# line/Human-Interaction-Generation

Measured on AMD Instinct MI355X. Metric: denoiser-fwd frames/s @ B=64·T=196, higher is better.
Workload: dtype f32; 1 GPU; MotionTransformer forward incl. the per-call cross-attention text side, BASELINE config 2: B=64/GPU T=196 F=150 d=512 L=8 H=8 ff=1024 N=77 Lt=256, linear attention, text embeddings supplied (CLIP stubbed); parallelism=dp1

## Files before the change

human-interaction-generation_amd/csrc/gemm_wsp32.hip:

```cpp
#include <stdlib.h>

#include <type_traits>

#include "hig_common.h"
#include "hig_host.h"

namespace {

typedef float f32x4 __attribute__((ext_vector_type(4)));
typedef int p32_i32x4 __attribute__((ext_vector_type(4)));

constexpr int P32_MAXSEG = HIG_P32_MAXSEG;
struct Wsp32Args {
  const float* X; int64_t ldx;
  const float* W; int64_t ldy;
  float* C; int64_t ldc;
  const float* res; int64_t ldr;
  float* aux; int64_t ldaux;
  const float* bias;
  int I, J;
  int ntiles;
  int nseg, seg_p0[P32_MAXSEG], seg_np[P32_MAXSEG];
  float* stats_out;
  const float* stats_in;
// ... 27 lines not shown
#if defined(__HIP_DEVICE_COMPILE__)
  const p32_i32x4 d = __builtin_bit_cast(p32_i32x4, v);
  if constexpr (POL == 1) __builtin_amdgcn_raw_buffer_store_b128(d, rs, byte_off, 0, 16);
  else __builtin_amdgcn_raw_buffer_store_b128(d, rs, byte_off, 0, 0);
#endif
}
__device__ __forceinline__ f32x4 p32_lds16(unsigned addr) {
  f32x4 v;
  asm volatile("ds_read_b128 %0, %1" : "=v"(v) : "v"(addr));
  return v;
}
typedef float f32x2_t __attribute__((ext_vector_type(2)));
__device__ __forceinline__ f32x2_t p32_lds8(unsigned addr) {
  f32x2_t v;
  asm volatile("ds_read_b64 %0, %1" : "=v"(v) : "v"(addr));
  return v;
}
__device__ __forceinline__ float p32_erf_abs(float ax, float& ex) {
  const float t = __builtin_amdgcn_rcpf(fmaf(ax, 0.3275911f * 0.70710678118654752440f, 1.0f));
  float p = fmaf(t, 1.061405429f, -1.453152027f);
  p = fmaf(t, p, 1.421413741f);
  p = fmaf(t, p, -0.284496736f);
  p = fmaf(t, p, 0.254829592f);
  p *= t;
  const float zz = ax * (0.70710678118654752440f * 1.2011224087864498f);
  ex = __builtin_amdgcn_exp2f(-(zz * zz));
  return fmaf(-p, ex, 1.0f);
}
__device__ __forceinline__ float p32_gelu(float x) {
  float ex;
  const float e = p32_erf_abs(fabsf(x), ex);
  return 0.5f * x * (1.0f + copysignf(e, x));
}
__device__ __forceinline__ float p32_dgelu(float z) {
  float ex;
  const float e = p32_erf_abs(fabsf(z), ex);
  return fmaf(z * 0.39894228040143267794f, ex, 0.5f + copysignf(0.5f * e, z));
}
__host__ __device__ constexpr bool p32_has_bias(int e) { return e == HIG_EPI_BIAS || e == HIG_EPI_BIAS_GELU || e == HIG_EPI_BIAS_RES; }
__host__ __device__ constexpr bool p32_has_res(int e) { return e == HIG_EPI_BIAS_RES || e == HIG_EPI_RES || e == HIG_EPI_DGELU; }

template <int PPR, int COUNT, int STEP>
__device__ __forceinline__ void p32_dma_rows([[maybe_unused]] __amdgpu_buffer_rsrc_t rs, int ld, int row0, int rmax, [[maybe_unused]] char* dst, int first, int lane) {
#pragma unroll
  for (int q = 0; q < COUNT; ++q) {
    const int n = first + STEP * q;
    const int r = n / PPR, part = n % PPR;
    [[maybe_unused]] const int voff = 16 * (lane ^ (r & 15));
    [[maybe_unused]] const int soff = min(row0 + r, rmax) * ld * 4 + part * 1024;
#if defined(__HIP_DEVICE_COMPILE__)
    __builtin_amdgcn_raw_ptr_buffer_load_lds(rs, (__attribute__((address_space(3))) void*)(dst + n * 1024), 16, voff, soff, 0, 0);
#endif
  }
}

template <int KW, int EPI, int XT, bool AUX, int POL, bool DIAG>
__global__ __launch_bounds__(512, 2) void gemm_wsp32_kernel(const Wsp32Args a) {
  constexpr int BM = 16;
  constexpr int ROWB = KW * 4;
  constexpr int XBUF = BM * ROWB;
  constexpr int RING = 128 * 1024;
  constexpr int NXB = RING / XBUF;
#ifndef P32_LOOK
#define P32_LOOK 1
#endif
  constexpr int LOOK = NXB - 1 < P32_LOOK ? NXB - 1 : P32_LOOK;
  constexpr bool NEED_CNT = NXB < LOOK + 2;
  constexpr int NH = KW / 256;
  constexpr int NC = 4 / NH;
  constexpr int BN = 32 * NC;
  constexpr int NKS = 16;
  constexpr int XS = 3;
  constexpr int RS = XS + 1;
  constexpr int HROW = BN * 4 + 16;
  constexpr int HPL = BM * HROW;
  constexpr int HBUF = NH * HPL;
  constexpr int RBUF = 4096, NRB = 3;
  constexpr int LBUF = 1024;
  constexpr int OFF_H = RING;
  constexpr int OFF_R = OFF_H + 2 * HBUF;
  constexpr int OFF_L = OFF_R + NRB * RBUF;
  constexpr int SMEM = OFF_L + (XT == 2 ? NRB * LBUF : 0);
  constexpr int OFF_C = OFF_H + BN * 4;
  constexpr int NSL = BN / 16;
  constexpr int PPR = ROWB / 1024;
  constexpr int NXI = BM * PPR / 4;
  constexpr int QPR = BN / 4;
  constexpr int RPP = QPR > 16 ? 64 / QPR : 4;
  constexpr int NPASS = 4 / RPP;
  constexpr bool HAS_RES = p32_has_res(EPI);
  static_assert(SMEM <= 160 * 1024, "LDS budget");
  static_assert(XT == 0 || (KW == 512 && ((XT == 1 && EPI == HIG_EPI_BIAS_RES) || (XT == 2 && EPI == HIG_EPI_BIAS))), "LayerNorm fold: K = 512, producer = BIAS_RES, consumer = BIAS");
  static_assert(!AUX || EPI == HIG_EPI_BIAS_GELU, "aux output: GELU epilogue only");
  static_assert(KW != 256 || (!HAS_RES && XT == 0 && !AUX), "K = 256 (the text-side key/value projection): plain / bias epilogue only");
  static_assert(NKS % RS == 0, "the ring index of a k-step is its number modulo RS in every tile");
  __shared__ __attribute__((aligned(1024))) char smem[160 * 1024];
  char* const sX = smem;
  char* const sH = smem + OFF_H;
  [[maybe_unused]] char* const sR = smem + OFF_R;
  [[maybe_unused]] char* const sL = smem + OFF_L;
  int* const scnt = reinterpret_cast<int*>(smem + OFF_C);

  const int tid = threadIdx.x, lane = tid & 63;
  const int wave = __builtin_amdgcn_readfirstlane(tid >> 6);
  const int w = (blockIdx.x & 7) * 32 + (blockIdx.x >> 3);
  constexpr bool W_BEHIND = KW == 512;
  static_assert(W_BEHIND ? (NSL == NXB && OFF_H + XBUF <= 160 * 1024) : NSL <= NXB, "weight slices fit");
  auto wslice = [&](int s) -> char* { return (W_BEHIND && s == NSL - 1) ? sH : sX + s * XBUF; };
  auto stamp = [&]([[maybe_unused]] int k) {
    if constexpr (!DIAG) return;
    if (a.stamps && (tid == 0 || tid == 256)) {
      unsigned long long tm;
      asm volatile("s_memtime %0\n\ts_waitcnt lgkmcnt(0)" : "=s"(tm)::"memory");
      a.stamps[(size_t)(tid ? 4096 : 0) + (size_t)blockIdx.x * 16 + k] = tm;
    }
  };
  stamp(0);

  if (wave < 4) {
    const int c = wave / NH, h = wave % NH;
    const int ln = lane & 15, kq = lane >> 4;
    int xo[4];
#pragma unroll
    for (int q = 0; q < 4; ++q) xo[q] = ln * ROWB + 1024 * h + 16 * ((4 * q + kq) ^ ln);
    const unsigned scnt_lds = (unsigned)(size_t)(__attribute__((address_space(3))) int*)scnt;
    const unsigned sx_lds = (unsigned)(size_t)(__attribute__((address_space(3))) char*)sX;
    char* const hmine = sH + h * HPL + ln * HROW + (32 * c + 4 * kq) * 4;

    for (int seg = 0; seg < a.nseg; ++seg) {
      const int nps = a.seg_np[seg], G = 256 / nps;
      const int rg = w / nps;
      const int tb = (int)((int64_t)rg * a.ntiles / G), te = (int)((int64_t)(rg + 1) * a.ntiles / G);
      const int nt = te - tb;
      p32_barrier();
      p32_barrier();
      f32x4 wf[NKS][2];
#pragma unroll
      for (int cb = 0; cb < 2; ++cb) {
        const char* wb = wslice(2 * c + cb);
#pragma unroll
        for (int ks = 0; ks < NKS; ++ks) wf[ks][cb] = *reinterpret_cast<const f32x4*>(wb + xo[ks & 3] + 256 * (ks >> 2));
      }
      p32_barrier();
      if (NEED_CNT && tid == 0) *scnt = 0;
      if (seg == 0) stamp(1);

      f32x4 acc0[2], acc1[2];
      f32x4 ring[RS];
#pragma unroll
      for (int e = 0; e < 2; ++e) { acc0[e] = f32x4{0.f, 0.f, 0.f, 0.f}; acc1[e] = f32x4{0.f, 0.f, 0.f, 0.f}; }
      auto signal_reads_issued = [&]() {
        if (lane == 0) asm volatile("ds_add_u32 %0, %1" ::"v"(scnt_lds), "v"(1) : "memory");
      };
      auto step = [&](auto has_tail, auto has_main, f32x4(&aP)[2], f32x4(&aQ)[2], int i) {
        constexpr bool TAIL = decltype(has_tail)::value, MAIN = decltype(has_main)::value;
        if (DIAG && seg == 0 && i == 5) stamp(11);
        if constexpr (TAIL && MAIN) asm volatile("s_waitcnt lgkmcnt(%0)" ::"n"(NEED_CNT ? XS + 1 : XS) : "memory");
        else asm volatile("s_waitcnt lgkmcnt(0)" ::: "memory");
        __builtin_amdgcn_s_barrier();
        asm volatile("" ::: "memory");
        if (DIAG && seg == 0 && i < 9) stamp(2 + i);
        unsigned xa[4];
        const unsigned xb = sx_lds + ((i + NXB - 1) % NXB) * XBUF;
#pragma unroll
        for (int q = 0; q < 4; ++q) {
          xa[q] = xb + xo[q];
          asm volatile("" : "+v"(xa[q]));
        }
        auto dump = [&]() {
          char* hp = hmine + ((i - 1) & 1) * HBUF;
#pragma unroll
          for (int cb = 0; cb < 2; ++cb) {
            *reinterpret_cast<f32x4*>(hp + cb * 64) = aQ[cb];
            aQ[cb] = f32x4{0.f, 0.f, 0.f, 0.f};
          }
        };
#pragma unroll
        for (int s = 0; s < NKS; ++s) {
#pragma unroll
          for (int j = 0; j < 4; ++j) {
#pragma unroll
            for (int cb = 0; cb < 2; ++cb) {
              if (s < XS) {
                if constexpr (TAIL) aQ[cb] = __builtin_amdgcn_mfma_f32_16x16x4f32(wf[NKS - XS + s][cb][j], ring[(NKS - XS + s) % RS][j], aQ[cb], 0, 0, 0);
              } else {
                if constexpr (MAIN) aP[cb] = __builtin_amdgcn_mfma_f32_16x16x4f32(wf[s - XS][cb][j], ring[(s - XS) % RS][j], aP[cb], 0, 0, 0);
              }
            }
            if constexpr (MAIN) {
              if (j == 0) ring[s % RS] = *reinterpret_cast<const __attribute__((address_space(3))) f32x4*>(xa[s & 3] + 256 * (s >> 2));
            }
          }
          if constexpr (TAIL) { if (s == (MAIN ? XS + 1 : XS - 1)) dump(); }
          {
            const int cur = (s < XS ? NKS - XS + s : s - XS) % RS;
            if ((s < XS && TAIL) || (s >= XS && MAIN)) asm volatile("" ::"v"(ring[cur]));
          }
          __builtin_amdgcn_sched_barrier(0);
        }
        if constexpr (MAIN && NEED_CNT) signal_reads_issued();
      };
      using T = std::true_type;
      using F = std::false_type;
      step(F{}, T{}, acc0, acc1, 0);
      int i = 1;
      for (; i + 1 < nt; i += 2) {
        step(T{}, T{}, acc1, acc0, i);
        step(T{}, T{}, acc0, acc1, i + 1);
      }
      if (i < nt) {
        step(T{}, T{}, acc1, acc0, i);
        ++i;
      }
      if (nt & 1) step(T{}, F{}, acc1, acc0, nt);
      else step(T{}, F{}, acc0, acc1, nt);
      p32_barrier();
    }
    stamp(12);
    return;
  }

  const int sw = wave - 4;
  const unsigned scnt_lds_s = (unsigned)(size_t)(__attribute__((address_space(3))) int*)scnt;
  if (a.prio == 1) __builtin_amdgcn_s_setprio(1);
  else if (a.prio == 2) __builtin_amdgcn_s_setprio(2);
  else if (a.prio == 3) __builtin_amdgcn_s_setprio(3);
  const int cq = lane & (QPR - 1), rsub = (lane / QPR) % RPP;
  const bool act = lane < 4 * QPR;
  __amdgpu_buffer_rsrc_t rsX = __builtin_amdgcn_make_buffer_rsrc(const_cast<float*>(a.X), 0, (int)(((int64_t)(a.I - 1) * a.ldx + KW) * 4), 0x00020000);
  __amdgpu_buffer_rsrc_t rsW = __builtin_amdgcn_make_buffer_rsrc(const_cast<float*>(a.W), 0, (int)(((int64_t)(a.J - 1) * a.ldy + KW) * 4), 0x00020000);
  __amdgpu_buffer_rsrc_t rsC = __builtin_amdgcn_make_buffer_rsrc(a.C, 0, (int)(((int64_t)(a.I - 1) * a.ldc + a.J) * 4), 0x00020000);
  [[maybe_unused]] __amdgpu_buffer_rsrc_t rsA = __builtin_amdgcn_make_buffer_rsrc(AUX ? a.aux : a.C, 0, (int)(((int64_t)(a.I - 1) * (AUX ? a.ldaux : a.ldc) + a.J) * 4), 0x00020000);
  [[maybe_unused]] __amdgpu_buffer_rsrc_t rsR = __builtin_amdgcn_make_buffer_rsrc(const_cast<float*>(HAS_RES ? a.res : a.X), 0, (int)(((int64_t)(a.I - 1) * (HAS_RES ? a.ldr : a.ldx) + (HAS_RES ? a.J : KW)) * 4), 0x00020000);
  for (int seg = 0; seg < a.nseg; ++seg) {
    const int nps = a.seg_np[seg], G = 256 / nps;
    const int panel = a.seg_p0[seg] + w % nps, rg = w / nps;
    const int tb = (int)((int64_t)rg * a.ntiles / G), te = (int)((int64_t)(rg + 1) * a.ntiles / G);
    const int nt = te - tb;
    const int j0 = panel * BN;
    f32x4 bq = {0.f, 0.f, 0.f, 0.f}, cs = {0.f, 0.f, 0.f, 0.f};
    auto dma_x = [&](int t) { p32_dma_rows<PPR, NXI, 4>(rsX, (int)a.ldx, (tb + t) * BM, a.I - 1, sX + ((t + NXB - 1) % NXB) * XBUF, sw, lane); };
    auto dma_res = [&](int t) {
      if constexpr (HAS_RES) {
        [[maybe_unused]] const int voff = (min((tb + t) * BM + 4 * sw + rsub, a.I - 1) * (int)a.ldr + j0 + 4 * cq) * 4;
#if defined(__HIP_DEVICE_COMPILE__)
        __builtin_amdgcn_raw_ptr_buffer_load_lds(rsR, (__attribute__((address_space(3))) void*)(sR + (t % NRB) * RBUF + sw * 1024), 16, voff, 0, 0, 0);
#endif
      }
    };
    auto dma_stats = [&](int t) {
      if constexpr (XT == 2) {
        if (sw == 0) {
          const int i = min((tb + t) * BM + (lane >> 2), a.I - 1);
          __builtin_amdgcn_global_load_lds((const __attribute__((address_space(1))) void*)(a.stats_in + (int64_t)i * 16 + 4 * (lane & 3)),
                                           (__attribute__((address_space(3))) void*)(sL + (t % NRB) * LBUF), 16, 0, 0);
        }
      }
    };

    p32_barrier();
#pragma unroll
    for (int s = 0; s < NSL; ++s) p32_dma_rows<PPR, NXI, 4>(rsW, (int)a.ldy, j0 + 16 * s, a.J - 1, wslice(s), sw, lane);
    if constexpr (p32_has_bias(EPI)) asm volatile("global_load_dwordx4 %0, %1, off" : "=v"(bq) : "v"(a.bias + j0 + 4 * cq) : "memory");
    if constexpr (XT == 2) asm volatile("global_load_dwordx4 %0, %1, off" : "=v"(cs) : "v"(a.colsum + j0 + 4 * cq) : "memory");
    int pre = 0;
    if constexpr (W_BEHIND) { dma_x(0); pre = 1; asm volatile("s_waitcnt vmcnt(%2)" : "+v"(bq), "+v"(cs) : "n"(NXI) : "memory"); }
    else asm volatile("s_waitcnt vmcnt(0)" : "+v"(bq), "+v"(cs) :: "memory");
    p32_barrier();
    p32_barrier();
    for (int t = pre; t < LOOK && t < nt; ++t) dma_x(t);
    {
      const int later = (max(min(LOOK, nt), 1) - 1) * NXI;
      p32_wait_vm(later);
    }

    constexpr int NST = NPASS * (1 + (XT == 1 ? 1 : 0) + (AUX ? 1 : 0));
    const unsigned sh_lds = (unsigned)(size_t)(__attribute__((address_space(3))) char*)sH;
    [[maybe_unused]] const unsigned sr_lds = (unsigned)(size_t)(__attribute__((address_space(3))) char*)sR;
    [[maybe_unused]] const unsigned sl_lds = (unsigned)(size_t)(__attribute__((address_space(3))) char*)sL;
    auto epilogue = [&](int e) {
#pragma unroll
     for (int pass = 0; pass < NPASS; ++pass) {
      const int row = 4 * sw + RPP * pass + rsub;
      const unsigned hp = sh_lds + (e & 1) * HBUF + row * HROW + 16 * cq;
      f32x4 hh[NH];
#pragma unroll
      for (int p = 0; p < NH; ++p) hh[p] = p32_lds16(hp + p * HPL);
      [[maybe_unused]] f32x4 rr = {0.f, 0.f, 0.f, 0.f};
      if constexpr (HAS_RES) rr = p32_lds16(sr_lds + (e % NRB) * RBUF + sw * 1024 + lane * 16);
      [[maybe_unused]] f32x2_t ps = {0.f, 0.f};
      if constexpr (XT == 2) ps = p32_lds8(sl_lds + (e % NRB) * LBUF + row * 64 + 8 * (cq & 7));
      if constexpr (NH == 1) asm volatile("s_waitcnt lgkmcnt(0)" : "+v"(hh[0]), "+v"(rr), "+v"(ps));
      else if constexpr (NH == 2) asm volatile("s_waitcnt lgkmcnt(0)" : "+v"(hh[0]), "+v"(hh[1]), "+v"(rr), "+v"(ps));
      else asm volatile("s_waitcnt lgkmcnt(0)" : "+v"(hh[0]), "+v"(hh[1]), "+v"(hh[2]), "+v"(hh[3]), "+v"(rr), "+v"(ps));
      float v[4];
#pragma unroll
      for (int k = 0; k < 4; ++k) {
        v[k] = hh[0][k];
#pragma unroll
        for (int p = 1; p < NH; ++p) v[k] += hh[p][k];
      }
      if constexpr (XT == 2) {
        const bool mine = cq < 8;
        const float tot = row16_sum(mine ? ps.x : 0.f), m2 = row16_sum(mine ? ps.y : 0.f);
        const float mean = tot * (1.0f / 512.0f);
        const float d0 = fmaf(ps.x, 1.0f / 64.0f, -mean);
        const float between = row16_sum(mine ? d0 * d0 : 0.f);
        const float rstd = rsqrtf(fmaf(64.0f, between, m2) * (1.0f / 512.0f) + 1e-5f), mr = -mean * rstd;
#pragma unroll
        for (int k = 0; k < 4; ++k) v[k] = fmaf(v[k], rstd, mr * cs[k]);
      }
#pragma unroll
      for (int k = 0; k < 4; ++k) v[k] += bq[k];
      const int ig = min((tb + e) * BM + row, a.I - 1);
      if constexpr (AUX) { if (act && !(DIAG && (a.dbg & 4))) p32_store16<POL>(rsA, (ig * (int)a.ldaux + j0 + 4 * cq) * 4, f32x4{v[0], v[1], v[2], v[3]}); }
#pragma unroll
      for (int k = 0; k < 4; ++k) {
        if constexpr (EPI == HIG_EPI_BIAS_RES || EPI == HIG_EPI_RES) v[k] += rr[k];
        if constexpr (EPI == HIG_EPI_BIAS_GELU) v[k] = p32_gelu(v[k]);
        if constexpr (EPI == HIG_EPI_DGELU) v[k] *= p32_dgelu(rr[k]);
      }
      if (DIAG && (a.dbg & 4)) { asm volatile("" ::"v"(v[0]), "v"(v[1]), "v"(v[2]), "v"(v[3])); continue; }
      if (act) p32_store16<POL>(rsC, (ig * (int)a.ldc + j0 + 4 * cq) * 4, f32x4{v[0], v[1], v[2], v[3]});
      if constexpr (XT == 1) {
        const float sm = row16_sum((v[0] + v[1]) + (v[2] + v[3]));
        const float pm = sm * (1.0f / 64.0f);
        const float a0 = v[0] - pm, a1 = v[1] - pm, a2 = v[2] - pm, a3 = v[3] - pm;
        const float qq = row16_sum((a0 * a0 + a1 * a1) + (a2 * a2 + a3 * a3));
        if (cq == 0) *reinterpret_cast<float2*>(a.stats_out + ((int64_t)ig * (a.J >> 6) + panel) * 2) = make_float2(sm, qq);
      }
     }
    };

    auto dbg = [&](int bit) { return DIAG && (a.dbg & bit) != 0; };
    auto n_x = [&](int i) { return (i >= 0 && i + LOOK < nt && !(dbg(1) && i > 2)) ? NXI : 0; };
    auto n_r = [&](int i) { return (HAS_RES && i >= 0 && i < nt) ? 1 : 0; };
    auto n_s = [&](int i) { return (XT == 2 && i >= 0 && i < nt && sw == 0) ? 1 : 0; };
    auto n_st = [&](int i) { return (i >= 2 && i < nt + 2 && !dbg(6)) ? NST : 0; };
    for (int i = 0; i < nt + 2; ++i) {
      p32_barrier();
      if (DIAG && i == 4 && seg == 0) stamp(0);
      if (i < nt) { dma_res(i); dma_stats(i); }
      if (DIAG && i == 4 && seg == 0) stamp(4);
      if (n_x(i)) {
        if constexpr (NEED_CNT) {
          int seen;
          do {
            asm volatile("ds_read_b32 %0, %1\n\ts_waitcnt lgkmcnt(0)" : "=v"(seen) : "v"(scnt_lds_s) : "memory");
          } while (__builtin_amdgcn_readfirstlane(seen) < 4 * i);
        }
        dma_x(i + LOOK);
      }
      if (DIAG && i == 4 && seg == 0) stamp(1);
      if (i >= 2 && !dbg(2)) epilogue(i - 2);
      if (DIAG && i == 4 && seg == 0) stamp(2);
      if constexpr (LOOK == 1) p32_wait_vm(n_st(i));
// ... 82 lines not shown
```

human-interaction-generation_amd/csrc/linattn.hip:

```cpp
#include <stdlib.h>

#include "hig_host.h"

namespace {

constexpr int CH = 64;

template <int HD> struct Patch {
  static constexpr int PC = HD >= 128 ? 8 : HD >= 64 ? 4 : HD >= 32 ? 2 : 1;
  static constexpr int PL = PC;
  static constexpr int TL = HD / PL;
};

template <int HD>
__global__ __launch_bounds__(256) void ctx_kernel(const float* __restrict__ K,
                                                  const float* __restrict__ V, int64_t ld, int rows,
                                                  int H, const int64_t* __restrict__ length,
                                                  float* __restrict__ A, float* __restrict__ kstat) {
  constexpr int LDP = HD + 4;
  constexpr int PC = Patch<HD>::PC, PL = Patch<HD>::PL, TL = Patch<HD>::TL;
  constexpr int RG = 256 / HD;
  __shared__ __attribute__((aligned(16))) float sP[CH * LDP];
  __shared__ __attribute__((aligned(16))) float sV[CH * LDP];
  __shared__ float sred[256];
// ... 1606 lines not shown
        const float dv = acc[hh][tb][e] - mean;
        qd += dv * dv;
      }
  }
  qd += __shfl_xor(qd, 32, 64);
  if (kk == 0) red[1][wave][lr] = qd;
  __syncthreads();
  const float rstd = rsqrtf(((red[1][0][lr] + red[1][1][lr]) + (red[1][2][lr] + red[1][3][lr])) / (float)d + 1e-5f);
  TO* sO = reinterpret_cast<TO*>(smem_dyn);
  const int ldso = d + 16 / (int)sizeof(TO);
  const float* ssrow = ss + (int64_t)b * ss_ld;
#pragma unroll
  for (int hh = 0; hh < MAXHPW; ++hh) {
    if (hh >= HPW) break;
    const int h = wave * HPW + hh;
#pragma unroll
    for (int tb = 0; tb < TB; ++tb)
#pragma unroll
      for (int qq = 0; qq < 4; ++qq) {
        const int col = h * HD + 32 * tb + 8 * qq + 4 * kk;
        const float4 g4 = *reinterpret_cast<const float4*>(gamma + col), b4 = *reinterpret_cast<const float4*>(beta + col);
        const float4 sc = *reinterpret_cast<const float4*>(ssrow + col), sh = *reinterpret_cast<const float4*>(ssrow + shift_off + col);
        float4 o;
        o.x = apply_sty_act<TO>(((acc[hh][tb][4 * qq] - mean) * rstd * g4.x + b4.x) * (1.0f + sc.x) + sh.x);
        o.y = apply_sty_act<TO>(((acc[hh][tb][4 * qq + 1] - mean) * rstd * g4.y + b4.y) * (1.0f + sc.y) + sh.y);
        o.z = apply_sty_act<TO>(((acc[hh][tb][4 * qq + 2] - mean) * rstd * g4.z + b4.z) * (1.0f + sc.z) + sh.z);
        o.w = apply_sty_act<TO>(((acc[hh][tb][4 * qq + 3] - mean) * rstd * g4.w + b4.w) * (1.0f + sc.w) + sh.w);
        st4(sO + lr * ldso + col, o);
      }
  }
  __syncthreads();
  constexpr int EO = 16 / (int)sizeof(TO);
  const int c16 = d / EO;
  for (int idx = tid; idx < 32 * c16; idx += 256) {
    const int rr = idx / c16, ch = idx % c16;
    if (r0 + rr < rows)
      *reinterpret_cast<uint4*>(Out + ((int64_t)b * rows + r0 + rr) * ldo + EO * ch) =
          *reinterpret_cast<const uint4*>(sO + rr * ldso + EO * ch);
  }
}

template <typename TQ, typename TO>
int launch_apply_sty(const TQ* q, int64_t ldq, const float* A, const float* gamma, const float* beta, const float* ss,
                     int64_t ss_ld, int32_t shift_off, TO* o, int64_t ldo, int32_t B, int32_t rows, int32_t H, int32_t hd,
                     hipStream_t st) {
  const int nblk = (rows + 31) / 32;
  const int d = H * hd;
  const size_t wbuf = (size_t)32 * (hd + 4) > 4096 ? (size_t)32 * (hd + 4) : 4096;
  const size_t lds_main = 4 * wbuf * sizeof(float);
  const size_t lds_out = (size_t)32 * (d + 16 / sizeof(TO)) * sizeof(TO);
  const size_t lds = lds_main > lds_out ? lds_main : lds_out;
  constexpr bool HAS64 = !std::is_same<TQ, float>::value;
  static const int big_lds_rc = [] {
    hipError_t e1 = hipSuccess;
    if constexpr (HAS64)
      e1 = hipFuncSetAttribute(reinterpret_cast<const void*>(&apply_sty_kernel<64, TQ, TO>),
                               hipFuncAttributeMaxDynamicSharedMemorySize, 156 * 1024);
    hipError_t e2 = hipFuncSetAttribute(reinterpret_cast<const void*>(&apply_sty_kernel<128, TQ, TO>),
                                        hipFuncAttributeMaxDynamicSharedMemorySize, 156 * 1024);
    return (e1 == hipSuccess && e2 == hipSuccess) ? 0 : 1;
  }();
  if (big_lds_rc != 0 || lds > 156 * 1024)
    return hig_set_error(HIG_EHIP, "hig_linattn_apply_sty: cannot reserve %zu bytes of LDS", lds);
  if (hd == 64) {
    if constexpr (HAS64)
      hipLaunchKernelGGL((apply_sty_kernel<64, TQ, TO>), dim3(B * nblk), dim3(256), lds, st, q, ldq, A, gamma, beta, ss, ss_ld,
                         shift_off, o, ldo, rows, H, nblk);
    else
      return hig_set_error(HIG_EUNSUPPORTED, "hig_linattn_apply_sty: head dim 64 has its own fp32 kernel");
  } else
    hipLaunchKernelGGL((apply_sty_kernel<128, TQ, TO>), dim3(B * nblk), dim3(256), lds, st, q, ldq, A, gamma, beta, ss, ss_ld,
                       shift_off, o, ldo, rows, H, nblk);
  HIG_CHECK_LAUNCH();
  return HIG_OK;
}

template <int H>
__global__ __launch_bounds__(64 * H, 4) void apply_sty_wave64_kernel(const float* __restrict__ Q, int64_t ldq, const float* __restrict__ A,
                                                                    const float* __restrict__ gamma, const float* __restrict__ beta,
                                                                    const float* __restrict__ ss, int64_t ss_ld, int shift_off,
                                                                    float* __restrict__ Out, int64_t ldo, int rows) {
  constexpr int HD = 64, D = H * HD;
  __shared__ __attribute__((aligned(16))) float sW[H * 16 * HD];
  __shared__ __attribute__((aligned(16))) float sP[4 * D];
  __shared__ float2 sR[2][H][16];
  const int tid = threadIdx.x, lane = tid & 63, h = tid >> 6;
  const int b = blockIdx.x;
  const int r = lane & 15, kq = lane >> 4;
  const int ntile = (rows + 15) >> 4, step = gridDim.y;
  const float* qb = Q + (int64_t)b * rows * ldq + h * HD + 16 * kq;
  la_f32x4 qt[4];
  auto fetch = [&](int tile, la_f32x4 (&v)[4]) {
    const int row = min(min(tile, ntile - 1) * 16 + r, rows - 1);
    const float* p = qb + (int64_t)row * ldq;
    asm volatile("global_load_dwordx4 %0, %4, off\n\tglobal_load_dwordx4 %1, %4, off offset:16\n\t"
                 "global_load_dwordx4 %2, %4, off offset:32\n\tglobal_load_dwordx4 %3, %4, off offset:48"
                 : "=&v"(v[0]), "=&v"(v[1]), "=&v"(v[2]), "=&v"(v[3]) : "v"(p) : "memory");
  };
  int tile = blockIdx.y;
  fetch(tile, qt);
  float aop[16][4];
  {
    const float4* Ab = reinterpret_cast<const float4*>(A + (((int64_t)b * H + h) * HD + 16 * kq) * HD) + r;
#pragma unroll
    for (int s2 = 0; s2 < 16; ++s2) {
      const float4 a4 = Ab[s2 * (HD / 4)];
      aop[s2][0] = a4.x; aop[s2][1] = a4.y; aop[s2][2] = a4.z; aop[s2][3] = a4.w;
    }
    const int arr = tid / (D / 4), idx = tid % (D / 4);
    const float* ssrow = ss + (int64_t)b * ss_ld;
    const float* src = arr == 0 ? gamma : arr == 1 ? beta : arr == 2 ? ssrow : ssrow + shift_off;
    float4 pv = *reinterpret_cast<const float4*>(src + 4 * idx);
    if (arr == 2) pv = make_float4(1.0f + pv.x, 1.0f + pv.y, 1.0f + pv.z, 1.0f + pv.w);
    *reinterpret_cast<float4*>(sP + arr * D + 4 * idx) = pv;
  }
  float* const so = sW + h * (16 * HD);
  __syncthreads();
  [[maybe_unused]] __amdgpu_buffer_rsrc_t rsO = __builtin_amdgcn_make_buffer_rsrc(Out + (int64_t)b * rows * ldo, 0, (int)(((int64_t)(rows - 1) * ldo + D) * 4), 0x00020000);
  int par = 0;
  auto tile_out = [&](int tile, auto younger) {
    la_f32x4 (&cur)[4] = qt;
    constexpr int YOUNGER = decltype(younger)::value;
    asm volatile("s_waitcnt vmcnt(%4)" : "+v"(cur[0]), "+v"(cur[1]), "+v"(cur[2]), "+v"(cur[3]) : "n"(YOUNGER) : "memory");
    float m = fmaxf(fmaxf(fmaxf(cur[0].x, cur[0].y), fmaxf(cur[0].z, cur[0].w)), fmaxf(fmaxf(cur[1].x, cur[1].y), fmaxf(cur[1].z, cur[1].w)));
    m = fmaxf(m, fmaxf(fmaxf(fmaxf(cur[2].x, cur[2].y), fmaxf(cur[2].z, cur[2].w)), fmaxf(fmaxf(cur[3].x, cur[3].y), fmaxf(cur[3].z, cur[3].w))));
    m = fmaxf(m, __shfl_xor(m, 16, 64));
    m = fmaxf(m, __shfl_xor(m, 32, 64));
    float p[16];
    float sum = 0.f;
#pragma unroll
    for (int i = 0; i < 4; ++i) {
      p[4 * i] = __expf(cur[i].x - m); p[4 * i + 1] = __expf(cur[i].y - m); p[4 * i + 2] = __expf(cur[i].z - m); p[4 * i + 3] = __expf(cur[i].w - m);
      sum += (p[4 * i] + p[4 * i + 1]) + (p[4 * i + 2] + p[4 * i + 3]);
    }
    sum += __shfl_xor(sum, 16, 64);
    sum += __shfl_xor(sum, 32, 64);
    const float inv = 1.0f / sum;
    la_f32x4 acc[4];
#pragma unroll
    for (int blk = 0; blk < 4; ++blk) acc[blk] = la_f32x4{0.f, 0.f, 0.f, 0.f};
#pragma unroll
    for (int s2 = 0; s2 < 16; ++s2) {
      const float ps = p[s2] * inv;
#pragma unroll
      for (int blk = 0; blk < 4; ++blk) acc[blk] = __builtin_amdgcn_mfma_f32_16x16x4f32(aop[s2][blk], ps, acc[blk], 0, 0, 0);
    }
    float bs = 0.f;
#pragma unroll
    for (int blk = 0; blk < 4; ++blk) bs += (acc[blk][0] + acc[blk][1]) + (acc[blk][2] + acc[blk][3]);
    bs += __shfl_xor(bs, 16, 64);
    bs += __shfl_xor(bs, 32, 64);
    const float bm = bs * (1.0f / HD);
    float bq = 0.f;
#pragma unroll
    for (int blk = 0; blk < 4; ++blk) {
      const float d0 = acc[blk][0] - bm, d1 = acc[blk][1] - bm, d2 = acc[blk][2] - bm, d3 = acc[blk][3] - bm;
      bq += (d0 * d0 + d1 * d1) + (d2 * d2 + d3 * d3);
    }
    bq += __shfl_xor(bq, 16, 64);
    bq += __shfl_xor(bq, 32, 64);
#pragma unroll
    for (int e = 0; e < 4; ++e)
      *reinterpret_cast<la_f32x4*>(so + r * HD + ((16 * kq + 4 * e) ^ (4 * r))) = la_f32x4{acc[0][e], acc[1][e], acc[2][e], acc[3][e]};
    if (kq == 0) sR[par][h][r] = make_float2(bs, bq);
    lds_barrier();
    float tot = 0.f, within = 0.f;
#pragma unroll
    for (int hh = 0; hh < H; ++hh) {
      const float2 ps = sR[par][hh][r];
      tot += ps.x; within += ps.y;
    }
    const float mean = tot * (1.0f / D);
    asm volatile("" ::: "memory");
    float between = 0.f;
#pragma unroll
    for (int hh = 0; hh < H; ++hh) {
      const float dm = fmaf(sR[par][hh][r].x, 1.0f / HD, -mean);
      between = fmaf(dm, dm, between);
    }
    par ^= 1;
    const float rstd = rsqrtf(fmaf((float)HD, between, within) * (1.0f / D) + 1e-5f);
#pragma unroll
    for (int e = 0; e < 4; ++e) {
      const int col = h * HD + 16 * kq + 4 * e;
      const float4 g4 = *reinterpret_cast<const float4*>(sP + col), b4 = *reinterpret_cast<const float4*>(sP + D + col);
      const float4 sc = *reinterpret_cast<const float4*>(sP + 2 * D + col), sh = *reinterpret_cast<const float4*>(sP + 3 * D + col);
      float* const yp = so + r * HD + ((16 * kq + 4 * e) ^ (4 * r));
      const float4 y4 = *reinterpret_cast<const float4*>(yp);
      float4 o;
      o.x = hig_silu(((y4.x - mean) * rstd * g4.x + b4.x) * sc.x + sh.x);
      o.y = hig_silu(((y4.y - mean) * rstd * g4.y + b4.y) * sc.y + sh.y);
      o.z = hig_silu(((y4.z - mean) * rstd * g4.z + b4.z) * sc.z + sh.z);
      o.w = hig_silu(((y4.w - mean) * rstd * g4.w + b4.w) * sc.w + sh.w);
      *reinterpret_cast<float4*>(yp) = o;
      asm volatile("" ::: "memory");
    }
    fetch(tile + step < ntile ? tile + step : tile, qt);
    asm volatile("s_waitcnt lgkmcnt(0)" ::: "memory");
#pragma unroll
    for (int i = 0; i < 4; ++i) {
      const int rr = 4 * i + kq, cc = 4 * r;
      [[maybe_unused]] const float4 v = *reinterpret_cast<const float4*>(so + rr * HD + (cc ^ (4 * rr)));
      [[maybe_unused]] const int row = tile * 16 + rr;
#if defined(__HIP_DEVICE_COMPILE__)
      __builtin_amdgcn_raw_buffer_store_b128(__builtin_bit_cast(la_i32x4, v), rsO, (row * (int)ldo + h * HD + cc) * 4, 0, 0);
#endif
    }
    asm volatile("s_waitcnt lgkmcnt(0)" ::: "memory");
  };
  tile_out(tile, std::integral_constant<int, 0>{});
  for (tile += step; tile < ntile; tile += step) tile_out(tile, std::integral_constant<int, 4>{});
  asm volatile("s_waitcnt vmcnt(0)" ::: "memory");
}

template <int H>
int launch_apply_sty_wave64(const float* q, int64_t ldq, const float* A, const float* gamma, const float* beta, const float* ss,
                            int64_t ss_ld, int32_t shift_off, float* o, int64_t ldo, int32_t B, int32_t rows, int nstrip, hipStream_t st) {
  hipLaunchKernelGGL((apply_sty_wave64_kernel<H>), dim3(B, nstrip), dim3(64 * H), 0, st, q, ldq, A, gamma, beta, ss, ss_ld, shift_off, o,
                     ldo, rows);
  HIG_CHECK_LAUNCH();
  return HIG_OK;
}

template <typename TIO>
int launch_apply_bwd(const hig_attn_plan_t& p, const TIO* dY, int64_t lddy, const TIO* Q, int64_t ldq, const float* A, TIO* dQ, int64_t lddq,
                     float* dA, int32_t B, int32_t rows, int32_t H, int32_t hd, float* scratch, hipStream_t st) {
  const bool merge = p.variant & HIG_ATTN_VARIANT_MERGE;
  if (p.path == HIG_ATTN_PATH_APPLY_BWD_MFMA) {
    with_mfma_hd(hd, [&](auto c) {
      hipLaunchKernelGGL((apply_bwd_mfma_kernel<HDC(c), TIO>), dim3(B * H, p.split), dim3(256), attn_bwd_lds_bytes<HDC(c)>(), st, dY, lddy, Q,
                         ldq, A, dQ, lddq, merge ? scratch : dA, rows, H);
    });
  } else if constexpr (sizeof(TIO) == 4) {
    HD_SWITCH(hd, hipLaunchKernelGGL((apply_bwd_kernel<HDV>), dim3(B * H, p.split), dim3(256), 0, st, dY, lddy, Q, ldq, A, dQ, lddq, scratch,
                                     rows, H));
  }
  HIG_CHECK_LAUNCH();
  if (!merge) return HIG_OK;
  const int64_t n = (int64_t)hd * hd, groups = (int64_t)B * H;
  const int64_t want = (groups * n / 4 + 255) / 256;
  hipLaunchKernelGGL(chunk_sum_kernel, dim3((unsigned)(want > 2048 ? 2048 : want)), dim3(256), 0, st, scratch, p.split, n, groups, dA);
  HIG_CHECK_LAUNCH();
  return HIG_OK;
}

template <typename TIO>
int launch_ctx_bwd(const hig_attn_plan_t& p, const float* dA, const float* A, const TIO* K, const TIO* V, int64_t ld, const float* kstat,
                   const int64_t* length, TIO* dK, TIO* dV, int64_t ldd, int32_t B, int32_t rows, int32_t H, int32_t hd, float* scratch,
                   hipStream_t st) {
  if (p.path == HIG_ATTN_PATH_CTX_BWD_MFMA) {
    with_mfma_hd(hd, [&](auto c) {
      hipLaunchKernelGGL((ctx_bwd_mfma_kernel<HDC(c), TIO>), dim3(B * H, p.split), dim3(256), attn_bwd_lds_bytes<HDC(c)>(), st, dA, A, K, V, ld,
                         kstat, length, dK, dV, ldd, rows, H);
    });
  } else if constexpr (sizeof(TIO) == 4) {
    HD_SWITCH(hd, hipLaunchKernelGGL((ctx_bwd_kernel<HDV>), dim3(B * H, p.split), dim3(256), 0, st, dA, K, V, ld, kstat, length, dK, dV, ldd,
                                     rows, H, scratch));
    HIG_CHECK_LAUNCH();
    HD_SWITCH(hd, hipLaunchKernelGGL((ctx_bwd_finish_kernel<HDV>), dim3(B * H, p.split), dim3(256), 0, st, K, ld, kstat, length, dK, ldd, rows,
                                     H, scratch));
  }
  HIG_CHECK_LAUNCH();
  return HIG_OK;
}

int plan_bwd_entry(hig_attn_plan_t* p, const hig_attn_call& c) {
  hig_attn_call aligned = c;
  aligned.facts |= HIG_ATTN_FACT_IN8 | HIG_ATTN_FACT_IN16 | HIG_ATTN_FACT_OUT8 | HIG_ATTN_FACT_OUT16;
  const bool would_use = c.hd == 128 && hig_attn_plan_for(aligned, hig_attn_switch_values(), hig_chip_cus(), true).rc == HIG_OK;
  return hig_attn_plan_entry(p, c, !would_use || allow_big_lds() == 0);
}
bool sty_out_i32(int64_t rows, int64_t ldo) { return rows <= 0 || ldo <= (INT32_MAX / 4) / (rows + 16); }

}

extern "C" int hig_linattn_ctx_bf16(const void* K, const void* V, int64_t ld, int32_t B, int32_t rows, int32_t H,
                                    int32_t hd, const int64_t* length, float* A, float* kstat, float* scratch,
                                    void* At16, hig_stream_t stream) {
  hig_attn_plan_t p;
  HIG_TRY(hig_attn_plan_entry(&p, {HIG_ATTN_ENTRY_CTX, HIG_ATTN_IO_BF16, B, rows, 0, H, hd, scratch != nullptr,
                              hig_attn_facts(K && V && A && kstat, row_bits<__bf16>(ld, K, V), 0)}));
  return launch_ctx<__bf16>(p, static_cast<const __bf16*>(K), static_cast<const __bf16*>(V), ld, B, rows, H, hd, length, A, kstat, scratch,
                            static_cast<__bf16*>(At16), hig_stream(stream));
}
extern "C" int hig_linattn_apply_bf16(const void* Q, int64_t ldq, const float* A, void* Y, int64_t ldy, int32_t B,
                                      int32_t rows, int32_t H, int32_t hd, hig_stream_t stream) {
  hig_attn_plan_t p;
  HIG_TRY(hig_attn_plan_entry(&p, {HIG_ATTN_ENTRY_APPLY, HIG_ATTN_IO_BF16, B, rows, 0, H, hd, false,
                              hig_attn_facts(Q && A && Y, row_bits<__bf16>(ldq, Q), row_bits<__bf16>(ldy, Y))}));
  return launch_apply<__bf16>(p, static_cast<const __bf16*>(Q), ldq, A, static_cast<__bf16*>(Y), ldy, B, rows, H, hd, hig_stream(stream));
}

extern "C" int64_t hig_linattn_bwd_scratch_floats(int32_t B, int32_t rows, int32_t H, int32_t hd) {
  const int64_t nchunk = (rows + CH - 1) / CH;
// ... 81 lines not shown
```

Baseline: 2.147 million frames/s.

## Load GEMM weights straight from global into MFMA-wave registers, skipping LDS staging

The compute waves now read their weight fragments directly from global memory into registers, instead of having the producer waves DMA the weight panel into LDS and then reading it back. This drops the two extra barriers and the weight-DMA phase, so the first X tile DMA can start right away, and it shrinks the LDS allocation to the computed size. Segments with no tiles now return early. The tradeoff is uncoalesced, strided global reads of W by each compute wave (row stride ldy) at the start of every segment, and a changed handshake between producer and consumer waves.

```diff
diff --git a/human-interaction-generation_amd/csrc/gemm_wsp32.hip b/human-interaction-generation_amd/csrc/gemm_wsp32.hip
--- a/human-interaction-generation_amd/csrc/gemm_wsp32.hip
+++ b/human-interaction-generation_amd/csrc/gemm_wsp32.hip
@@ -133,7 +133,6 @@
   constexpr int OFF_L = OFF_R + NRB * RBUF;
   constexpr int SMEM = OFF_L + (XT == 2 ? NRB * LBUF : 0);
   constexpr int OFF_C = OFF_H + BN * 4;
-  constexpr int NSL = BN / 16;
   constexpr int PPR = ROWB / 1024;
   constexpr int NXI = BM * PPR / 4;
   constexpr int QPR = BN / 4;
@@ -145,7 +144,7 @@
   static_assert(!AUX || EPI == HIG_EPI_BIAS_GELU, "aux output: GELU epilogue only");
   static_assert(KW != 256 || (!HAS_RES && XT == 0 && !AUX), "K = 256 (the text-side key/value projection): plain / bias epilogue only");
   static_assert(NKS % RS == 0, "the ring index of a k-step is its number modulo RS in every tile");
-  __shared__ __attribute__((aligned(1024))) char smem[160 * 1024];
+  __shared__ __attribute__((aligned(1024))) char smem[SMEM];
   char* const sX = smem;
   char* const sH = smem + OFF_H;
   [[maybe_unused]] char* const sR = smem + OFF_R;
@@ -155,9 +154,6 @@
   const int tid = threadIdx.x, lane = tid & 63;
   const int wave = __builtin_amdgcn_readfirstlane(tid >> 6);
   const int w = (blockIdx.x & 7) * 32 + (blockIdx.x >> 3);
-  constexpr bool W_BEHIND = KW == 512;
-  static_assert(W_BEHIND ? (NSL == NXB && OFF_H + XBUF <= 160 * 1024) : NSL <= NXB, "weight slices fit");
-  auto wslice = [&](int s) -> char* { return (W_BEHIND && s == NSL - 1) ? sH : sX + s * XBUF; };
   auto stamp = [&]([[maybe_unused]] int k) {
     if constexpr (!DIAG) return;
     if (a.stamps && (tid == 0 || tid == 256)) {
@@ -180,21 +176,22 @@
 
     for (int seg = 0; seg < a.nseg; ++seg) {
       const int nps = a.seg_np[seg], G = 256 / nps;
-      const int rg = w / nps;
+      const int panel = a.seg_p0[seg] + w % nps, rg = w / nps;
       const int tb = (int)((int64_t)rg * a.ntiles / G), te = (int)((int64_t)(rg + 1) * a.ntiles / G);
       const int nt = te - tb;
-      p32_barrier();
-      p32_barrier();
+      if (nt == 0) { p32_barrier(); continue; }
       f32x4 wf[NKS][2];
-#pragma unroll
-      for (int cb = 0; cb < 2; ++cb) {
-        const char* wb = wslice(2 * c + cb);
-#pragma unroll
-        for (int ks = 0; ks < NKS; ++ks) wf[ks][cb] = *reinterpret_cast<const f32x4*>(wb + xo[ks & 3] + 256 * (ks >> 2));
-      }
+      {
+        const float* wr = a.W + (int64_t)(panel * BN + 32 * c + ln) * a.ldy + 256 * h + 4 * kq;
+#pragma unroll
+        for (int ks = 0; ks < NKS; ++ks) {
+#pragma unroll
+          for (int cb = 0; cb < 2; ++cb) wf[ks][cb] = *reinterpret_cast<const f32x4*>(wr + (int64_t)(16 * cb) * a.ldy + 16 * ks);
+        }
+      }
+      if (seg == 0) stamp(1);
       p32_barrier();
       if (NEED_CNT && tid == 0) *scnt = 0;
-      if (seg == 0) stamp(1);
 
       f32x4 acc0[2], acc1[2];
       f32x4 ring[RS];
@@ -250,6 +247,10 @@
           __builtin_amdgcn_sched_barrier(0);
         }
         if constexpr (MAIN && NEED_CNT) signal_reads_issued();
+        if constexpr (!TAIL) {
+#pragma unroll
+          for (int s = NKS - XS; s < NKS; ++s) asm volatile("" ::"v"(wf[s][0]), "v"(wf[s][1]));
+        }
       };
       using T = std::true_type;
       using F = std::false_type;
@@ -279,7 +280,6 @@
   const int cq = lane & (QPR - 1), rsub = (lane / QPR) % RPP;
   const bool act = lane < 4 * QPR;
   __amdgpu_buffer_rsrc_t rsX = __builtin_amdgcn_make_buffer_rsrc(const_cast<float*>(a.X), 0, (int)(((int64_t)(a.I - 1) * a.ldx + KW) * 4), 0x00020000);
-  __amdgpu_buffer_rsrc_t rsW = __builtin_amdgcn_make_buffer_rsrc(const_cast<float*>(a.W), 0, (int)(((int64_t)(a.J - 1) * a.ldy + KW) * 4), 0x00020000);
   __amdgpu_buffer_rsrc_t rsC = __builtin_amdgcn_make_buffer_rsrc(a.C, 0, (int)(((int64_t)(a.I - 1) * a.ldc + a.J) * 4), 0x00020000);
   [[maybe_unused]] __amdgpu_buffer_rsrc_t rsA = __builtin_amdgcn_make_buffer_rsrc(AUX ? a.aux : a.C, 0, (int)(((int64_t)(a.I - 1) * (AUX ? a.ldaux : a.ldc) + a.J) * 4), 0x00020000);
   [[maybe_unused]] __amdgpu_buffer_rsrc_t rsR = __builtin_amdgcn_make_buffer_rsrc(const_cast<float*>(HAS_RES ? a.res : a.X), 0, (int)(((int64_t)(a.I - 1) * (HAS_RES ? a.ldr : a.ldx) + (HAS_RES ? a.J : KW)) * 4), 0x00020000);
@@ -309,20 +309,16 @@
       }
     };
 
-    p32_barrier();
-#pragma unroll
-    for (int s = 0; s < NSL; ++s) p32_dma_rows<PPR, NXI, 4>(rsW, (int)a.ldy, j0 + 16 * s, a.J - 1, wslice(s), sw, lane);
+    if (nt == 0) { p32_barrier(); continue; }
+    dma_x(0);
     if constexpr (p32_has_bias(EPI)) asm volatile("global_load_dwordx4 %0, %1, off" : "=v"(bq) : "v"(a.bias + j0 + 4 * cq) : "memory");
     if constexpr (XT == 2) asm volatile("global_load_dwordx4 %0, %1, off" : "=v"(cs) : "v"(a.colsum + j0 + 4 * cq) : "memory");
-    int pre = 0;
-    if constexpr (W_BEHIND) { dma_x(0); pre = 1; asm volatile("s_waitcnt vmcnt(%2)" : "+v"(bq), "+v"(cs) : "n"(NXI) : "memory"); }
-    else asm volatile("s_waitcnt vmcnt(0)" : "+v"(bq), "+v"(cs) :: "memory");
     p32_barrier();
-    p32_barrier();
-    for (int t = pre; t < LOOK && t < nt; ++t) dma_x(t);
+    for (int t = 1; t < LOOK && t < nt; ++t) dma_x(t);
     {
       const int later = (max(min(LOOK, nt), 1) - 1) * NXI;
       p32_wait_vm(later);
+      asm volatile("" : "+v"(bq), "+v"(cs));
     }
 
     constexpr int NST = NPASS * (1 + (XT == 1 ? 1 : 0) + (AUX ? 1 : 0));
```

Result: no change. 2.146 million frames/s (median of 3 runs) (-0.0%).

## Stream Q tiles into LDS via buffer-load-to-LDS DMA in apply_sty wave64 kernel

Applied to the files above, without the earlier changes.

Replaces the per-thread global loads of Q into registers with buffer_load-to-LDS DMA into a new swizzled shared buffer. The next tile's DMA is issued right after the current tile is read back from LDS, rather than at the end of the tile. The gamma/beta/scale-shift and A-operand loads become hand-issued asm loads, with explicit vmcnt waits placed so they overlap the first tile's softmax. The initial block barrier is removed and the parameter staging is folded into the first tile. This is meant to hide global load latency and cut VGPR pressure, at the cost of extra LDS per block (possibly lower occupancy) and fragile hand-counted waitcnt ordering.

```diff
diff --git a/human-interaction-generation_amd/csrc/linattn.hip b/human-interaction-generation_amd/csrc/linattn.hip
--- a/human-interaction-generation_amd/csrc/linattn.hip
+++ b/human-interaction-generation_amd/csrc/linattn.hip
@@ -1712,46 +1712,62 @@
                                                                     float* __restrict__ Out, int64_t ldo, int rows) {
   constexpr int HD = 64, D = H * HD;
   __shared__ __attribute__((aligned(16))) float sW[H * 16 * HD];
+  __shared__ __attribute__((aligned(16))) float sQ[H * 16 * HD];
   __shared__ __attribute__((aligned(16))) float sP[4 * D];
   __shared__ float2 sR[2][H][16];
-  const int tid = threadIdx.x, lane = tid & 63, h = tid >> 6;
+  const int tid = threadIdx.x, lane = tid & 63;
+  const int h = __builtin_amdgcn_readfirstlane(tid >> 6);
   const int b = blockIdx.x;
   const int r = lane & 15, kq = lane >> 4;
   const int ntile = (rows + 15) >> 4, step = gridDim.y;
-  const float* qb = Q + (int64_t)b * rows * ldq + h * HD + 16 * kq;
-  la_f32x4 qt[4];
-  auto fetch = [&](int tile, la_f32x4 (&v)[4]) {
-    const int row = min(min(tile, ntile - 1) * 16 + r, rows - 1);
-    const float* p = qb + (int64_t)row * ldq;
-    asm volatile("global_load_dwordx4 %0, %4, off\n\tglobal_load_dwordx4 %1, %4, off offset:16\n\t"
-                 "global_load_dwordx4 %2, %4, off offset:32\n\tglobal_load_dwordx4 %3, %4, off offset:48"
-                 : "=&v"(v[0]), "=&v"(v[1]), "=&v"(v[2]), "=&v"(v[3]) : "v"(p) : "memory");
+  const int arr = tid / (D / 4), idx = tid % (D / 4);
+  la_f32x4 pv;
+  {
+    const float* ssrow = ss + (int64_t)b * ss_ld;
+    const float* src = (arr == 0 ? gamma : arr == 1 ? beta : arr == 2 ? ssrow : ssrow + shift_off) + 4 * idx;
+    asm volatile("global_load_dwordx4 %0, %1, off" : "=v"(pv) : "v"(src) : "memory");
+  }
+  [[maybe_unused]] __amdgpu_buffer_rsrc_t rsQ = __builtin_amdgcn_make_buffer_rsrc(const_cast<float*>(Q + (int64_t)b * rows * ldq), 0, (int)(((int64_t)(rows - 1) * ldq + D) * 4), 0x00020000);
+  [[maybe_unused]] char* const qdst = reinterpret_cast<char*>(sQ + h * (16 * HD));
+  [[maybe_unused]] const int ldq4 = (int)ldq * 4, qcol = h * (HD * 4) + 16 * (r ^ kq);
+  auto dma = [&]([[maybe_unused]] int tile) {
+#pragma unroll
+    for (int j = 0; j < 4; ++j) {
+      [[maybe_unused]] const int voff = min(tile * 16 + 4 * j + kq, rows - 1) * ldq4 + (qcol ^ (64 * j));
+#if defined(__HIP_DEVICE_COMPILE__)
+      __builtin_amdgcn_raw_ptr_buffer_load_lds(rsQ, (__attribute__((address_space(3))) void*)(qdst + j * 1024), 16, voff, 0, 0, 0);
+#endif
+    }
   };
   int tile = blockIdx.y;
-  fetch(tile, qt);
-  float aop[16][4];
+  dma(tile);
+  la_f32x4 aop[16];
   {
-    const float4* Ab = reinterpret_cast<const float4*>(A + (((int64_t)b * H + h) * HD + 16 * kq) * HD) + r;
-#pragma unroll
-    for (int s2 = 0; s2 < 16; ++s2) {
-      const float4 a4 = Ab[s2 * (HD / 4)];
-      aop[s2][0] = a4.x; aop[s2][1] = a4.y; aop[s2][2] = a4.z; aop[s2][3] = a4.w;
-    }
-    const int arr = tid / (D / 4), idx = tid % (D / 4);
-    const float* ssrow = ss + (int64_t)b * ss_ld;
-    const float* src = arr == 0 ? gamma : arr == 1 ? beta : arr == 2 ? ssrow : ssrow + shift_off;
-    float4 pv = *reinterpret_cast<const float4*>(src + 4 * idx);
-    if (arr == 2) pv = make_float4(1.0f + pv.x, 1.0f + pv.y, 1.0f + pv.z, 1.0f + pv.w);
-    *reinterpret_cast<float4*>(sP + arr * D + 4 * idx) = pv;
+    const float* Ab = A + (((int64_t)b * H + h) * HD + 16 * kq) * HD + 4 * r;
+#define STY_LDA(s2) asm volatile("global_load_dwordx4 %0, %1, off offset:%2" : "=v"(aop[s2]) : "v"(Ab), "n"((s2) * HD * 4) : "memory")
+    STY_LDA(0); STY_LDA(1); STY_LDA(2); STY_LDA(3); STY_LDA(4); STY_LDA(5); STY_LDA(6); STY_LDA(7);
+    STY_LDA(8); STY_LDA(9); STY_LDA(10); STY_LDA(11); STY_LDA(12); STY_LDA(13); STY_LDA(14); STY_LDA(15);
+#undef STY_LDA
   }
   float* const so = sW + h * (16 * HD);
-  __syncthreads();
+  const unsigned qrd = (unsigned)(size_t)(__attribute__((address_space(3))) char*)sQ + h * (16 * HD * 4) + r * (HD * 4);
   [[maybe_unused]] __amdgpu_buffer_rsrc_t rsO = __builtin_amdgcn_make_buffer_rsrc(Out + (int64_t)b * rows * ldo, 0, (int)(((int64_t)(rows - 1) * ldo + D) * 4), 0x00020000);
   int par = 0;
-  auto tile_out = [&](int tile, auto younger) {
-    la_f32x4 (&cur)[4] = qt;
-    constexpr int YOUNGER = decltype(younger)::value;
-    asm volatile("s_waitcnt vmcnt(%4)" : "+v"(cur[0]), "+v"(cur[1]), "+v"(cur[2]), "+v"(cur[3]) : "n"(YOUNGER) : "memory");
+  auto tile_out = [&](int tile, auto first) {
+    constexpr bool FIRST = decltype(first)::value;
+    la_f32x4 cur[4];
+    if constexpr (FIRST) {
+      asm volatile("s_waitcnt vmcnt(%1)" : "+v"(pv) : "n"(16) : "memory");
+      if (arr == 2) pv = la_f32x4{1.0f + pv.x, 1.0f + pv.y, 1.0f + pv.z, 1.0f + pv.w};
+      *reinterpret_cast<la_f32x4*>(sP + arr * D + 4 * idx) = pv;
+    } else {
+      asm volatile("s_waitcnt vmcnt(%0)" : : "n"(4) : "memory");
+    }
+#pragma unroll
+    for (int i = 0; i < 4; ++i) asm volatile("ds_read_b128 %0, %1" : "=v"(cur[i]) : "v"(qrd + 16 * ((4 * kq + i) ^ r)));
+    asm volatile("s_waitcnt lgkmcnt(0)" : "+v"(cur[0]), "+v"(cur[1]), "+v"(cur[2]), "+v"(cur[3]) : : "memory");
+    dma(tile + step < ntile ? tile + step : tile);
+    __builtin_amdgcn_sched_barrier(0);
     float m = fmaxf(fmaxf(fmaxf(cur[0].x, cur[0].y), fmaxf(cur[0].z, cur[0].w)), fmaxf(fmaxf(cur[1].x, cur[1].y), fmaxf(cur[1].z, cur[1].w)));
     m = fmaxf(m, fmaxf(fmaxf(fmaxf(cur[2].x, cur[2].y), fmaxf(cur[2].z, cur[2].w)), fmaxf(fmaxf(cur[3].x, cur[3].y), fmaxf(cur[3].z, cur[3].w))));
     m = fmaxf(m, __shfl_xor(m, 16, 64));
@@ -1766,6 +1782,11 @@
     sum += __shfl_xor(sum, 16, 64);
     sum += __shfl_xor(sum, 32, 64);
     const float inv = 1.0f / sum;
+    if constexpr (FIRST) {
+      __builtin_amdgcn_sched_barrier(0);
+      asm volatile("s_waitcnt vmcnt(%8)" : "+v"(aop[0]), "+v"(aop[1]), "+v"(aop[2]), "+v"(aop[3]), "+v"(aop[4]), "+v"(aop[5]), "+v"(aop[6]), "+v"(aop[7]) : "n"(4) : "memory");
+      asm volatile("s_waitcnt vmcnt(%8)" : "+v"(aop[8]), "+v"(aop[9]), "+v"(aop[10]), "+v"(aop[11]), "+v"(aop[12]), "+v"(aop[13]), "+v"(aop[14]), "+v"(aop[15]) : "n"(4) : "memory");
+    }
     la_f32x4 acc[4];
 #pragma unroll
     for (int blk = 0; blk < 4; ++blk) acc[blk] = la_f32x4{0.f, 0.f, 0.f, 0.f};
@@ -1825,7 +1846,6 @@
       *reinterpret_cast<float4*>(yp) = o;
       asm volatile("" ::: "memory");
     }
-    fetch(tile + step < ntile ? tile + step : tile, qt);
     asm volatile("s_waitcnt lgkmcnt(0)" ::: "memory");
 #pragma unroll
     for (int i = 0; i < 4; ++i) {
@@ -1838,8 +1858,8 @@
     }
     asm volatile("s_waitcnt lgkmcnt(0)" ::: "memory");
   };
-  tile_out(tile, std::integral_constant<int, 0>{});
-  for (tile += step; tile < ntile; tile += step) tile_out(tile, std::integral_constant<int, 4>{});
+  tile_out(tile, std::true_type{});
+  for (tile += step; tile < ntile; tile += step) tile_out(tile, std::false_type{});
   asm volatile("s_waitcnt vmcnt(0)" ::: "memory");
 }
 
```

Result: no change. 2.131 million frames/s before, 2.151 million frames/s after, median of 6 (+0.9%).
